# ucsdarclab/diffco

Hardware: AMD Instinct MI355X
Metric: million collision-score+grad evals/sec, 7-DoF FK-kernel, 2k supports (higher is better)
Workload: dtype f32

## Files before the change

diffco_amd/_lib.py:

```python
import ctypes as C
import os

import torch

from ._fkdesc import FkDesc

_HERE = os.path.dirname(os.path.abspath(__file__))
LIB_PATH = os.environ.get("DCX_LIB") or os.path.join(_HERE, "libdcx.so")

_c_fp = C.c_void_p
SYMBOLS = {
    "dcx_version": (C.c_int, []),
    "dcx_last_error": (C.c_char_p, []),
    "dcx_device_count": (C.c_int, []),
    "dcx_debug_set": (C.c_int, [C.c_char_p, C.c_int64]),
    "dcx_debug_clock_probe": (C.c_int, [C.c_int, C.c_void_p, C.c_uint64, C.POINTER(C.c_int32), C.c_void_p]),
    "dcx_model_create": (C.c_int, [C.POINTER(C.c_void_p), C.c_int, C.POINTER(FkDesc), C.c_int, C.POINTER(C.c_float),
                                   _c_fp, _c_fp, C.c_int64, C.c_int32, C.c_int32]),
    "dcx_model_create_ex": (C.c_int, [C.POINTER(C.c_void_p), C.c_int, C.POINTER(FkDesc), C.c_int, C.POINTER(C.c_float),
                                      _c_fp, _c_fp, C.c_int64, C.c_int32, C.c_int32, C.c_int64, C.c_void_p]),
    "dcx_model_update": (C.c_int, [C.c_void_p, _c_fp, _c_fp, C.c_int64, C.c_void_p]),
    "dcx_model_destroy": (None, [C.c_void_p]),
    "dcx_model_info": (C.c_int, [C.c_void_p, C.POINTER(C.c_int64), C.POINTER(C.c_int32), C.POINTER(C.c_int32),
                                 C.POINTER(C.c_int32), C.POINTER(C.c_int32)]),
    "dcx_score": (C.c_int, [C.c_void_p, _c_fp, C.c_int64, _c_fp, C.c_void_p]),
    "dcx_score_grad": (C.c_int, [C.c_void_p, _c_fp, C.c_int64, _c_fp, _c_fp, _c_fp, C.c_void_p]),
    "dcx_score_jac": (C.c_int, [C.c_void_p, _c_fp, C.c_int64, _c_fp, _c_fp, C.c_void_p]),
    "dcx_score_hess": (C.c_int, [C.c_void_p, _c_fp, C.c_int64, _c_fp, _c_fp, _c_fp, C.c_void_p]),
    "dcx_score_hinge_grad": (C.c_int, [C.c_void_p, _c_fp, C.c_int64, C.c_float, C.c_float, _c_fp, _c_fp, C.c_void_p]),
    "dcx_score_hinge_grad_mc": (C.c_int, [C.c_void_p, _c_fp, C.c_int64, C.POINTER(C.c_float), C.c_float, _c_fp, _c_fp, C.c_void_p]),
    "dcx_traj_adam_run_mc": (C.c_int, [C.c_void_p, C.c_void_p, C.c_void_p, C.POINTER(C.c_float), C.c_int32, C.c_int32, C.c_void_p]),
    "dcx_traj_adam_step_mc": (C.c_int, [C.c_int, C.POINTER(FkDesc), C.c_void_p, C.c_void_p, C.POINTER(C.c_float), C.c_int32, C.c_int32,
                                        C.c_void_p]),
    "dcx_traj_adam_step": (C.c_int, [C.c_int, C.POINTER(FkDesc), C.c_void_p, C.c_void_p, C.c_int32, C.c_void_p]),
    "dcx_traj_adam_run": (C.c_int, [C.c_void_p, C.c_void_p, C.c_void_p, C.c_int32, C.c_int32, C.c_void_p]),
    "dcx_escape_work_bytes": (C.c_size_t, [C.c_void_p, C.c_int64]),
    "dcx_escape_adam": (C.c_int, [C.c_void_p, _c_fp, C.c_int64, _c_fp, C.c_void_p, C.c_void_p, C.c_size_t, _c_fp, C.c_void_p,
                                  C.c_void_p]),
    "dcx_train_perceptron": (C.c_int, [C.c_int, C.c_int, C.POINTER(C.c_float), C.c_float, _c_fp, C.c_int64, C.c_int32, _c_fp,
                                       C.c_int32, _c_fp, _c_fp, _c_fp, C.c_int32, _c_fp, C.c_void_p]),
    "dcx_train_perceptron_ex": (C.c_int, [C.c_int, C.c_int, C.POINTER(C.c_float), C.c_float, _c_fp, C.c_int64, C.c_int32, _c_fp,
                                          C.c_int32, _c_fp, _c_fp, _c_fp, C.c_int32, _c_fp, C.c_int32, C.c_void_p]),
    "dcx_fkine": (C.c_int, [C.c_int, C.POINTER(FkDesc), _c_fp, C.c_int64, _c_fp, C.c_void_p]),
    "dcx_fkine_vjp": (C.c_int, [C.c_int, C.POINTER(FkDesc), _c_fp, _c_fp, C.c_int64, _c_fp, C.c_void_p]),
    "dcx_dh_frames": (C.c_int, [C.c_int, _c_fp, C.c_int64, C.c_int32, _c_fp, _c_fp, _c_fp, _c_fp, _c_fp, C.c_void_p]),
    "dcx_dh_frames_vjp": (C.c_int, [C.c_int, _c_fp, C.c_int64, C.c_int32, _c_fp, _c_fp, _c_fp, _c_fp, _c_fp, C.c_void_p]),
    "dcx_euler_frames": (C.c_int, [C.c_int, _c_fp, C.c_int64, _c_fp, C.c_void_p]),
    "dcx_euler_frames_vjp": (C.c_int, [C.c_int, _c_fp, _c_fp, C.c_int64, _c_fp, C.c_void_p]),
    "dcx_kernel_matrix": (C.c_int, [C.c_int, C.c_int, C.POINTER(C.c_float), _c_fp, C.c_int64, _c_fp, C.c_int64,
                                    C.c_int32, _c_fp, C.c_void_p]),
    "dcx_motion_work_bytes": (C.c_size_t, [C.c_void_p, C.c_int64]),
    "dcx_check_motions": (C.c_int, [C.c_void_p, _c_fp, _c_fp, C.c_int64, C.c_void_p, _c_fp, _c_fp, _c_fp, C.c_void_p, C.c_size_t,
                                    C.c_void_p]),
    "dcx_motion_cost_work_bytes": (C.c_size_t, [C.c_void_p, C.c_int64, C.c_int32]),
    "dcx_motion_cost": (C.c_int, [C.c_void_p, _c_fp, _c_fp, C.c_int64, C.c_void_p, _c_fp, C.c_float, _c_fp, _c_fp, _c_fp, _c_fp,
                                  C.c_void_p, C.c_size_t, C.c_void_p]),
    "dcx_solve_work_bytes": (C.c_size_t, [C.c_int64, C.c_int64]),
    "dcx_solve": (C.c_int, [C.c_int, _c_fp, _c_fp, C.c_int64, C.c_int64, _c_fp, C.c_void_p, C.c_size_t, C.c_void_p, C.c_int32,
                            C.c_void_p]),
}



class TrajState(C.Structure):
    _fields_ = [("n_paths", C.c_int32), ("n_waypoints", C.c_int32)] + [
        (n, C.c_void_p) for n in ("path", "adam_m", "adam_v", "limits", "col_score", "col_grad", "stats", "lowest_loss",
                                  "lowest_obj", "lowest_path", "best_valid_obj", "best_valid_path", "done", "steps")]

# ... 67 lines not shown
```

diffco_amd/csrc/dcx_api.hip:

```cpp
#include <algorithm>
#include <atomic>
#include <cmath>
#include <cstdio>
#include <cstdlib>
#include <cstring>
#include <mutex>
#include <new>
#include <string>
#include <vector>

#include "dcx_internal.h"
#include "motion_cost_kernel.h"
#include "motion_kernel.h"
#include "pack_kernels.h"
#include "solve_kernels.h"

using namespace dcx;

struct dcx_model {
    int device = 0;
    dcx_fk_desc fk{};
    FkProg* fk_dev = nullptr;
    DhProg* dh_dev = nullptr;
    DhArgs dh{};
// ... 182 lines not shown
}

int set_device(int device) {
    int n = 0;
    hipError_t e = hipGetDeviceCount(&n);
    if (e != hipSuccess || n == 0) return fail(DCX_ERR_NO_DEVICE, "no HIP device visible (libdcx has no CPU path)");
    if (device < 0 || device >= n) return fail(DCX_ERR_INVALID, "device index out of range");
    DCX_HIP(hipSetDevice(device));
    return DCX_OK;
}

struct FkCacheEntry {
    int device;
    dcx_fk_desc host;
    FkProg* dev;
};
thread_local std::vector<FkCacheEntry> g_fk_cache;

int upload_fk_prog(const dcx_fk_desc& fk, FkProg** out) {
    FkProg prog;
    build_fk_prog(fk, prog);
    FkProg* d = nullptr;
    DCX_HIP(hipMalloc((void**)&d, sizeof(FkProg)));
    hipError_t e = hipMemcpy(d, &prog, sizeof(FkProg), hipMemcpyHostToDevice);
    if (e != hipSuccess) {
        (void)hipFree(d);
        return fail_hip(e, "upload of the FK program");
    }
    *out = d;
    return DCX_OK;
}

int fk_device_copy(int device, const dcx_fk_desc& fk, FkProg** out) {
    for (auto& e : g_fk_cache)
        if (e.device == device && std::memcmp(&e.host, &fk, sizeof(fk)) == 0) {
            *out = e.dev;
            return DCX_OK;
        }
    FkProg* d = nullptr;
    if (int rc = upload_fk_prog(fk, &d)) return rc;
    if (g_fk_cache.size() >= 64) {
        (void)hipFree(g_fk_cache.front().dev);
        g_fk_cache.erase(g_fk_cache.begin());
    }
    g_fk_cache.push_back({device, fk, d});
    *out = d;
    return DCX_OK;
}

struct Knobs {
    std::atomic<int64_t> ys{-1}, nw{-1}, min_rows{-1}, split_finish_kernel{-1}, inlaunch_tiles{-1}, jac_per_class{-1},
        traj_fused{-1}, xf{-1}, jac_one_sweep{-1}, train_grid{-1}, fkk{-1}, jt_waves{-1}, hess_ys{-1}, hess_form{-1},
        traj_ys{-1}, traj_across{-1}, owner_poll{-1}, solve_threads{-1}, qt{-1}, giveup_inject{-1}, skew{-1}, skew8{-1},
        motion_early_exit{-1};
    Knobs() {
        auto rd = [](const char* name, std::atomic<int64_t>& dst, bool flag) {
            if (const char* e = std::getenv(name)) dst = flag ? 1 : std::atoll(e);
        };
        rd("DCX_YS", ys, false);
        rd("DCX_NW", nw, false);
        rd("DCX_MIN_ROWS", min_rows, false);
        rd("DCX_SPLIT_FINISH_KERNEL", split_finish_kernel, true);
        rd("DCX_INLAUNCH_TILES", inlaunch_tiles, false);
        rd("DCX_JAC_PER_CLASS", jac_per_class, true);
        rd("DCX_TRAJ_FUSED", traj_fused, false);
        rd("DCX_XF", xf, false);
        rd("DCX_JAC_ONE_SWEEP", jac_one_sweep, false);
        rd("DCX_TRAIN_GRID", train_grid, false);
        rd("DCX_FKK", fkk, false);
        rd("DCX_JT_WAVES", jt_waves, false);
        rd("DCX_HESS_YS", hess_ys, false);
        rd("DCX_HESS_FORM", hess_form, false);
        rd("DCX_TRAJ_YS", traj_ys, false);
        rd("DCX_TRAJ_ACROSS", traj_across, false);
        rd("DCX_OWNER_POLL", owner_poll, false);
        rd("DCX_SOLVE_THREADS", solve_threads, false);
        rd("DCX_QT", qt, false);
        rd("DCX_SKEW", skew, false);
        rd("DCX_SKEW8", skew8, false);
    }
};
Knobs& knobs() {
    static Knobs k;
    return k;
}

struct Geometry {
    int nw, ys;
    int red_slots;
};
Geometry pick_geometry(const dcx_model* m, int64_t B, int acc_floats, bool allow_split) {
    const int cap = m->max_threads / 64;
    const int64_t tiles = (B + 63) / 64;
    Geometry g;
    g.ys = 1;
    if (allow_split && 2 * tiles <= m->n_cu) {
        const int64_t want = std::min<int64_t>((int64_t)m->n_cu / tiles, m->S_active / 250);
        while (2 * g.ys <= want && g.ys < 32) g.ys *= 2;
        g.nw = std::min(16, cap);
    } else if (allow_split && 3 * tiles <= 2 * (int64_t)m->n_cu && (int64_t)m->S_active * m->Dt >= 18000) {
        g.ys = 3;
        g.nw = std::min(16, cap);
    } else {
        g.nw = std::min((tiles <= 4 * (int64_t)m->n_cu) ? 16 : 8, cap);
    }
    const Knobs& kn = knobs();
    if (const int64_t v = kn.ys; v >= 1 && allow_split) g.ys = (int)std::min<int64_t>(v, 64);
    if (const int64_t v = kn.nw; v >= 1) g.nw = (int)std::min<int64_t>(v, cap);
    int min_rows = 15;
    if (const int64_t v = kn.min_rows; v >= 1) min_rows = (int)v;
    while (g.ys > 1 && m->S_active / (g.ys * g.nw) < min_rows) g.ys /= 2;
    while (g.nw > 1 && m->S_active / (g.ys * g.nw) < min_rows) g.nw /= 2;
    const int d_fk = m->fk.n_points * m->fk.point_dim;
    auto lds_bytes = [&](int nw, int slots) {
        return (size_t)(lds_plan(m->fk.dof, d_fk, m->frame_floats, nw > 1 ? slots : 0, acc_floats, true).total + m->prog_floats) * sizeof(float);
    };
    g.red_slots = g.nw;
    const size_t lds_cap = (g.ys > 1 ? 150 : 64) * 1024;
    if (lds_bytes(g.nw, g.nw) > lds_cap && g.nw >= 8 && lds_bytes(g.nw / 2, g.nw / 2) <= lds_cap && kn.nw < 1) {
        g.nw /= 2;
        g.red_slots = g.nw;
    }
    if (lds_bytes(g.nw, g.nw) > lds_cap) {
        const int wps = sweep_min_waves(m->Dt, m->Cc, m->kf);
        int best_nw = 1, best_waves = 0;
        for (int nw = g.nw; nw >= 1; nw /= 2) {
            const size_t lds = lds_bytes(nw, 1);
            if (lds > 64 * 1024) continue;
            const int by_lds = (int)((160 * 1024) / lds), by_regs = std::max(1, (4 * wps) / nw);
            const int waves = std::min(by_lds, by_regs) * nw;
            if (waves > best_waves) {
                best_waves = waves;
                best_nw = nw;
            }
        }
        g.nw = best_nw;
        g.red_slots = 1;
    }
// ... 92 lines not shown
    }
    m->hess_mom.push_back({st, p, bytes});
    return p;
}

inline int32_t skew_rule(int Cc = 1, bool score_only = false, bool traj = false) {
    const int64_t k = knobs().skew;
    if (k >= 0) return (int32_t)k;
    if (traj && Cc > 1) return 340 | (300 << 10) | (240 << 20);
    if (score_only) return 320 | (300 << 10) | (240 << 20);
    return Cc > 1 ? (420 | (300 << 10) | (200 << 20)) : (480 | (320 << 10) | (150 << 20));
}

inline int32_t skew8_rule(bool score_only = false) {
    const int64_t k = knobs().skew8;
    if (k >= 0) return -(int32_t)k;
    if (score_only) return -540;
    return -600;
}

void set_fk_walk(const dcx_model* m, ScoreArgs& a) {
    a.fk = m->fk_dev;
    a.fk_dwords = m->fk_dwords;
    a.dh = m->dh;
    a.fkk = 0;
    if (m->fk.kind == DCX_FK_DH) {
        const int64_t k = knobs().fkk;
        a.fkk = (k == 0) ? 0 : (k == 1) ? 1 : (m->dh_dev ? 2 : 1);
    }
}

struct Hinge {
    int on = 0;
    float margin = 0.f, weight = 0.f;
    float margin_c[DCX_MAX_C] = {0.f, 0.f, 0.f, 0.f, 0.f, 0.f, 0.f, 0.f};
    int traj_slices = 0;
};

int run_score(const dcx_model* m, const float* q, int64_t B, const float* upstream, float* score, float* grad,
              int mode, int one_hot, int64_t grad_stride, hipStream_t st, Hinge hinge = Hinge(), int nz = 1) {
    if (B == 0) return DCX_OK;
    const int d_fk = m->fk.n_points * m->fk.point_dim;
    const int acc = (mode == MODE_SCORE ? 0 : m->Dt) + m->Cc;
    int64_t nblk = (B + 63) / 64;
    const bool xf_able = knobs().xf != 0 && xf_applies(m->Dt, m->Cc, m->kf) && m->rows_xf_dev != nullptr &&
                         (m->kf != KF_RQ2 || m->xf_rq_ok || knobs().xf >= 2);
    constexpr int QT_SLICES = kQtSlices;
    Geometry g{};
    bool qt = false;
    int qt_per = 0;
    size_t qt_lds = 0;
    const Knobs& kn0 = knobs();
    const bool asked_otherwise = kn0.ys >= 1 || kn0.xf >= 0 || kn0.owner_poll >= 0 || kn0.split_finish_kernel > 0 ||
                                 kn0.inlaunch_tiles >= 0 || kn0.min_rows >= 1;
    if (const int64_t kq = kn0.qt; kq != 0 && (kq > 0 || !asked_otherwise) && qt_applies(m->Dt, m->Cc, m->kf, mode) && nz == 1 &&
                                   m->S_active >= 64 && B <= 16LL * m->n_cu) {
        int nw = std::min(16, m->max_threads / 64);
        if (const int64_t v = knobs().nw; v >= 2) nw = (int)std::min<int64_t>(v, m->max_threads / 64);
        const int nw_rule = nw;
        for (; nw >= 4; nw /= 2) {
            qt_per = (m->S_active + QT_SLICES * nw - 1) / (QT_SLICES * nw);
            const size_t plan = lds_plan(m->fk.dof, d_fk, m->frame_floats, nw, acc, true).total + m->prog_floats;
            qt_lds = sizeof(float) * (((plan + 3) & ~(size_t)3) + (size_t)QT_SLICES * nw * (qt_per * row_stride(m->Dt, m->Cc) + 4) +
                                      (size_t)(12 * m->dh.n_pt + 1) * 64);
            if (qt_lds <= 156 * 1024 && qt_per >= 2) break;
            if (kq < 0) { nw = 0; break; }
        }
        if (nw >= 4 && (kq > 0 || nw == nw_rule)) {
            qt = true;
            g.nw = nw;
            g.ys = 1;
            g.red_slots = nw;
        }
    }
    if (!qt) g = pick_geometry(m, B * nz, acc, true);
    float* part = nullptr;
    uint32_t ptag = 0;
    if (knobs().giveup_inject > 0 && m->giveup_host) {
        knobs().giveup_inject = -1;
        *m->giveup_host = 1;
    }
    if (m->giveup_host && *m->giveup_host)
        return fail(DCX_ERR_HIP, "an earlier split launch of this model gave up waiting for its peer workgroups (owner-polls hand-over: "
                                 "they were never scheduled - the GPU is shared with another process?); its results were NaN. "
                                 "dcx_debug_set(\"owner_poll\", 0) selects the hand-over that never waits");
    if (g.ys > 1) {
        part = split_scratch(m, st, (size_t)nblk * nz * g.ys * acc * 64 * sizeof(float), &ptag);
        if (!part) g = pick_geometry(m, B * nz, acc, false);
    }
    unsigned int* counters = nullptr;
    if (part) {
        const bool second_launch = knobs().split_finish_kernel > 0;
        int64_t inlaunch_max = 256;
        if (const int64_t v = knobs().inlaunch_tiles; v >= 0) inlaunch_max = std::min<int64_t>(v, (int64_t)kTileCounters);
        if (nblk * nz <= inlaunch_max && !second_launch) counters = reinterpret_cast<unsigned int*>(part);
        part = reinterpret_cast<float*>(reinterpret_cast<char*>(part) + kScratchHead);
    }
    if (nblk > 0x7fffffffLL) return fail(DCX_ERR_UNSUPPORTED, "batch too large for one launch");
    ScoreArgs a{};
    a.rows = m->rows_dev;
    set_fk_walk(m, a);
    a.q = q;
    a.upstream = upstream;
    a.score = score;
    a.grad = grad;
    a.B = B;
    a.S = m->S_active;
// ... 11 lines not shown
    a.red_slots = g.red_slots;
    a.dof = m->fk.dof;
    a.d_fk = d_fk;
    a.frame_floats = m->frame_floats;
    a.kind = m->kind;
    a.c_out = m->C;
    a.one_hot = one_hot;
    a.nz = nz;
    a.grad_stride = grad_stride;
    a.kp0 = m->kp0_sweep;
    a.kp1 = m->kp1;
    a.hinge = hinge.on;
    a.hinge_margin = hinge.margin;
    a.hinge_weight = hinge.weight;
    for (int c = 0; c < DCX_MAX_C; ++c) a.hinge_margin_c[c] = hinge.margin_c[c];
    a.xf = xf_able ? 1 : 0;
    if (qt) {
        a.xf = 0;
        a.qt = 1;
        a.qt_per = qt_per;
        for (int gq = 0; gq < 4; ++gq) a.qt_per_g[gq] = qt_per;
        if (g.nw == 16 && skew_rule() > 0) {
            const int32_t sk = skew_rule();
            const int w3[3] = {sk & 1023, (sk >> 10) & 1023, (sk >> 20) & 1023};
            int left = 4 * qt_per;
            for (int gq = 0; gq < 3; ++gq) {
                a.qt_per_g[gq] = std::min(left, (int)((int64_t)4 * qt_per * w3[gq] / 1000));
                left -= a.qt_per_g[gq];
            }
            a.qt_per_g[3] = left;
        }
        a.qt_off = (int32_t)((lds_plan(a.dof, d_fk, m->frame_floats, g.nw, acc, true).total + m->prog_floats + 3) & ~3);
        a.qt_scr = a.qt_off + QT_SLICES * g.nw * (qt_per * row_stride(m->Dt, m->Cc) + 4);
        const int64_t kq = knobs().qt;
        a.qt_front = (int32_t)((int64_t)QT_SLICES * g.nw * qt_per * (kq >= 100 ? std::min<int64_t>(kq - 100, 100) : 45) / 100);
        nblk = (B + 15) / 16;
    }
    if (a.xf) {
        a.rows = m->rows_xf_dev;
        a.centre = m->centre_dev;
    }
    a.jt_rows = (a.fkk == 2 && g.nw >= 2 * m->dh.n_chains && m->dh.n_chains <= 2 && m->dh.end0 <= kDhUnroll &&
                 m->dh.n_steps - m->dh.end0 <= kDhUnroll && knobs().jt_waves != 0) ? 1 : 0;
    a.jt_waves = (a.jt_rows && mode != MODE_SCORE && g.red_slots == g.nw && (g.nw - 1) * acc >= 12 * m->dh.n_pt + 1 &&
                  (g.ys == 1 || counters != nullptr)) ? 1 : 0;
#ifdef DCX_TIMING
    if (!g_ts_dev && hipMalloc((void**)&g_ts_dev, sizeof(unsigned long long) * kTsWords) == hipSuccess)
        (void)hipMemset(g_ts_dev, 0, sizeof(unsigned long long) * kTsWords);
    a.ts = g_ts_dev;
    a.ts_block = std::getenv("DCX_TS_BLOCK") ? (unsigned)std::atoi(std::getenv("DCX_TS_BLOCK")) : 0u;
#endif
    size_t lds = sizeof(float) * (lds_plan(a.dof, d_fk, m->frame_floats, g.nw > 1 ? g.red_slots : 0, acc, true).total + m->prog_floats);
    if (qt) lds = qt_lds;
    if (g.ys == 1) {
        hipError_t e = m->launch(m->kf, m->Cc, mode, g.nw, lds, nblk, a, st);
        if (e != hipSuccess) return fail_hip(e, "score kernel launch");
        return DCX_OK;
    }
    if (nz > 1 && counters == nullptr) return DCX_ERR_UNSUPPORTED;
    a.partial = part;
    a.tile_done = counters;
    if (counters != nullptr && g.red_slots == g.nw && g.nw > 1 && knobs().owner_poll != 0 && (acc <= 2 * g.nw || knobs().owner_poll > 0) &&
        nblk * nz * g.ys <= (int64_t)m->n_cu && 2 * nblk * nz <= (int64_t)m->n_cu && m->giveup_dev != nullptr &&
        (knobs().owner_poll > 0 || opoll_stream_ok(m->device, st))) {
        a.pwords = reinterpret_cast<unsigned long long*>(reinterpret_cast<char*>(part) + (size_t)2 * m->n_cu * (m->Dt + m->Cc) * 64 * sizeof(float));
        a.ptag = ptag;
        a.giveup = m->giveup_dev;
    }
    hipError_t e = m->launch(m->kf, m->Cc, mode, g.nw, lds, nblk, a, st);
    if (e == hipSuccess && counters == nullptr) {
        FinishArgs f{};
        f.partial = part;
        f.fk = m->fk_dev;
        f.q = q;
        f.upstream = (m->C == 1) ? upstream : nullptr;
        f.score = score;
        f.grad = grad;
        f.B = B;
        f.grad_stride = grad_stride;
        f.ys = g.ys;
        f.acc = acc;
        f.C = m->Cc;
        f.c_out = m->C;
        f.Dt = m->Dt;
        f.dof = m->fk.dof;
        f.d_fk = d_fk;
        f.frame_floats = m->frame_floats;
        f.want_grad = (mode != MODE_SCORE);
        f.hinge = hinge.on;
        f.hinge_margin = hinge.margin;
        f.hinge_weight = hinge.weight;
        e = launch_score_finish(f, nblk, sizeof(float) * (lds_plan(a.dof, d_fk, m->frame_floats, 0, 0).total + m->prog_floats), st);
    }
    if (e != hipSuccess) return fail_hip(e, "split score launch");
    return DCX_OK;
}

}

extern "C" {

#ifdef DCX_TIMING
int dcx_debug_ts_words(void) { return (int)kTsWords; }
int dcx_debug_read_ts(unsigned long long* out) {
    if (!g_ts_dev) return 1;
    (void)hipDeviceSynchronize();
    return hipMemcpy(out, g_ts_dev, sizeof(unsigned long long) * kTsWords, hipMemcpyDeviceToHost) == hipSuccess ? 0 : 3;
}
#endif

int dcx_version(void) { return DCX_VERSION; }

int dcx_debug_set(const char* name, int64_t value) {
    if (!name) return fail(DCX_ERR_INVALID, "knob name is NULL");
    Knobs& k = knobs();
    const std::string n(name);
    if (n == "mfma" || n == "xm")
        return value > 0 ? fail(DCX_ERR_UNSUPPORTED, "the matrix-core forms of the sweep were removed (measured slower, profiles/r03_mfma_ab.txt)")
                         : DCX_OK;
    std::atomic<int64_t>* dst = n == "ys" ? &k.ys : n == "nw" ? &k.nw : n == "min_rows" ? &k.min_rows
        : n == "split_finish_kernel" ? &k.split_finish_kernel : n == "inlaunch_tiles" ? &k.inlaunch_tiles
        : n == "jac_per_class" ? &k.jac_per_class : n == "traj_fused" ? &k.traj_fused : n == "xf" ? &k.xf : n == "jac_one_sweep" ? &k.jac_one_sweep : n == "train_grid" ? &k.train_grid : n == "fkk" ? &k.fkk : n == "jt_waves" ? &k.jt_waves : n == "hess_ys" ? &k.hess_ys : n == "hess_form" ? &k.hess_form : n == "traj_ys" ? &k.traj_ys : n == "traj_across" ? &k.traj_across : n == "owner_poll" ? &k.owner_poll : n == "solve_threads" ? &k.solve_threads : n == "qt" ? &k.qt : n == "giveup_inject" ? &k.giveup_inject : n == "skew" ? &k.skew : n == "skew8" ? &k.skew8 : n == "motion_early_exit" ? &k.motion_early_exit : nullptr;
    if (!dst) return fail(DCX_ERR_INVALID, "unknown knob: " + n);
    *dst = value;
    return DCX_OK;
}

const char* dcx_last_error(void) { return g_err.c_str(); }

int dcx_device_count(void) {
    int n = 0;
    if (hipGetDeviceCount(&n) != hipSuccess) return 0;
    return n;
}

static constexpr double kXfRqRule = 32.0;
static size_t rows_tail_floats(const dcx_model* m) { return 8 * (size_t)m->RS + 16; }

static void model_free_rows(dcx_model* m) {
    if (m->rows_dev) (void)hipFree(m->rows_dev);
    if (m->rows_xf_dev) (void)hipFree(m->rows_xf_dev);
    if (m->rows_p2_dev) (void)hipFree(m->rows_p2_dev);
    m->rows_dev = m->rows_xf_dev = m->rows_p2_dev = nullptr;
    m->cap = 0;
}

static int model_alloc_rows(dcx_model* m, int64_t cap) {
    if (cap < 1) cap = 1;
    if (cap <= m->cap && m->rows_dev) return DCX_OK;
    const size_t floats = (size_t)cap * m->RS + rows_tail_floats(m);
    float *rows = nullptr, *rows_xf = nullptr, *rows_p2 = nullptr;
    hipError_t e = hipMalloc((void**)&rows, floats * sizeof(float));
    if (e == hipSuccess) e = hipMalloc((void**)&rows_xf, floats * sizeof(float));
    if (e == hipSuccess && p2_applies(m->Dt, m->Cc, m->kf)) e = hipMalloc((void**)&rows_p2, (floats + m->RS) * sizeof(float));
    if (e == hipSuccess && !m->centre_dev) e = hipMalloc((void**)&m->centre_dev, (size_t)m->Dt * sizeof(float));
    if (e == hipSuccess && !m->info_dev) e = hipMalloc((void**)&m->info_dev, 16);
    if (e == hipSuccess && !m->info_host) e = hipHostMalloc((void**)&m->info_host, 16, hipHostMallocDefault);
    if (e == hipSuccess && !m->giveup_host) {
        e = hipHostMalloc((void**)&m->giveup_host, sizeof(int32_t), hipHostMallocMapped);
        if (e == hipSuccess) {
            *m->giveup_host = 0;
            e = hipHostGetDevicePointer((void**)&m->giveup_dev, m->giveup_host, 0);
        }
    }
    if (e != hipSuccess) {
        if (rows) (void)hipFree(rows);
        if (rows_xf) (void)hipFree(rows_xf);
        if (rows_p2) (void)hipFree(rows_p2);
        return fail_hip(e, "device allocation of the model");
    }
    model_free_rows(m);
    m->rows_dev = rows;
    m->rows_xf_dev = rows_xf;
    m->rows_p2_dev = rows_p2;
    m->cap = cap;
    return DCX_OK;
}
// ... 1155 lines not shown
```

diffco_amd/csrc/score_inst.hip:

```cpp
#include "dcx_internal.h"
#include "traj_fused.h"
#include "jac_kernel.h"

#ifndef DCX_INST_D
#error "compile with -DDCX_INST_D=<feature width>"
#endif

#if (defined(DCX_STUB) && DCX_INST_PART != 0) || (DCX_INST_PART == 2 && DCX_INST_D > 24)
#elif defined(DCX_STUB)
namespace dcx {
#define DCX_CAT_(a, b) a##b
#define DCX_CAT(a, b) DCX_CAT_(a, b)
hipError_t DCX_CAT(launch_score_D, DCX_INST_D)(int, int, int, int, size_t, int64_t, const ScoreArgs&, hipStream_t) { return hipErrorNotSupported; }
hipError_t DCX_CAT(launch_jac_D, DCX_INST_D)(int, int, int, size_t, int64_t, const ScoreArgs&, hipStream_t) { return hipErrorNotSupported; }
hipError_t DCX_CAT(launch_traj_fused_D, DCX_INST_D)(int, int, int, size_t, int, const TrajFusedArgs&, hipStream_t) { return hipErrorNotSupported; }
}
#else
namespace dcx {
namespace {

constexpr int kD = DCX_INST_D;
constexpr int kMaxT = kD <= 16 ? 1024 : (kD <= 48 ? 512 : 256);


template <int KF, int CC, int MODE>
hipError_t go(int nw, size_t lds, int64_t nblk, const ScoreArgs& a, hipStream_t st) {
    const dim3 grid((unsigned)nblk, (unsigned)(a.ys > 1 ? a.ys : 1), (unsigned)(a.nz > 1 ? a.nz : 1));
    auto launch = [&](auto kern) {
        if (lds > 64 * 1024) {
            hipError_t e = hipFuncSetAttribute((const void*)kern, hipFuncAttributeMaxDynamicSharedMemorySize, (int)lds);
            if (e != hipSuccess) return e;
        }
        kern<<<grid, dim3(64 * nw), lds, st>>>(a);
        return hipGetLastError();
    };
    if constexpr (qt_applies(kD, CC, KF, MODE)) {
        if (a.qt) return launch(score_kernel<kD, KF, CC, MODE, kMaxT, false, true>);
    }
    if constexpr (xf_applies(kD, CC, KF)) {
        if (a.xf) return launch(score_kernel<kD, KF, CC, MODE, kMaxT, true>);
    }
    return launch(score_kernel<kD, KF, CC, MODE, kMaxT>);
}

template <int KF, int CC>
hipError_t by_mode(int mode, int nw, size_t lds, int64_t nblk, const ScoreArgs& a, hipStream_t st) {
    switch (mode) {
    case MODE_SCORE: return go<KF, CC, MODE_SCORE>(nw, lds, nblk, a, st);
    case MODE_GRAD_ROW: return go<KF, CC, MODE_GRAD_ROW>(nw, lds, nblk, a, st);
    case MODE_GRAD_UP:
        if constexpr (CC > 1) return go<KF, CC, MODE_GRAD_UP>(nw, lds, nblk, a, st);
    default: return hipErrorInvalidValue;
    }
}

template <int KF>
hipError_t by_cc(int cc, int mode, int nw, size_t lds, int64_t nblk, const ScoreArgs& a, hipStream_t st) {
    switch (cc) {
    case 1: return by_mode<KF, 1>(mode, nw, lds, nblk, a, st);
    case 5: return by_mode<KF, 5>(mode, nw, lds, nblk, a, st);
#ifndef DCX_DEV_FAST
    case 4: return by_mode<KF, 4>(mode, nw, lds, nblk, a, st);
    case 8: return by_mode<KF, 8>(mode, nw, lds, nblk, a, st);
#endif
    default: return hipErrorInvalidValue;
    }
}

}

#define DCX_CAT_(a, b) a##b
#define DCX_CAT(a, b) DCX_CAT_(a, b)
#ifndef DCX_INST_PART
#error "compile with -DDCX_INST_PART=0, 1 and (D <= 24) 2"
#endif
hipError_t DCX_CAT(launch_score_gen_D, DCX_INST_D)(int cc, int mode, int nw, size_t lds, int64_t nblk, const ScoreArgs& a, hipStream_t st);
namespace {
template <class K>
hipError_t traj_go(K kern, int nw, size_t lds, int n_paths, const TrajFusedArgs& a, hipStream_t st) {
    if (lds > 64 * 1024) {
        hipError_t e = hipFuncSetAttribute((const void*)kern, hipFuncAttributeMaxDynamicSharedMemorySize, (int)lds);
        if (e != hipSuccess) return e;
    }
    if (a.ys > 1) {
        TrajFusedArgs copy = a;
        void* params[] = {&copy};
        const dim3 grid = a.cl_across ? dim3((unsigned)a.ys, (unsigned)n_paths) : dim3((unsigned)n_paths, (unsigned)a.ys);
        return hipLaunchCooperativeKernel((const void*)kern, grid, dim3(64 * nw), params, (unsigned int)lds, st);
// ... 135 lines not shown
```

diffco_amd/csrc/score_kernel.h:

```cpp
#pragma once
#include <hip/hip_runtime.h>
#include <type_traits>
#include <stdint.h>
#include "fk_device.h"

namespace dcx {

enum { KF_RQ2 = 0,
       KF_POLY1 = 1,
       KF_GEN = 2 };

enum { MODE_SCORE = 0,
       MODE_GRAD_ROW = 1,
       MODE_GRAD_UP = 2 };

struct ScoreArgs {
    const float* rows;
    const float* centre;
    const FkProg* fk;
    const float* q;
    const float* upstream;
    float* score;
    float* grad;
    int64_t B;
    int32_t S;
    int32_t s_chunk;
    int32_t dof;
    int32_t d_fk;
    int32_t frame_floats;
    int32_t kind;
    int32_t c_out;
    int32_t one_hot;
    int32_t nz;
    int64_t grad_stride;
    float* partial;
    unsigned int* tile_done;
    unsigned long long* pwords;
    uint32_t ptag;
    int32_t* giveup;
    int32_t ys;
    int32_t s_super;
    int32_t red_slots;
#ifdef DCX_TIMING
    unsigned long long* ts;
    unsigned int ts_block;
#endif
    float kp0, kp1;
    int32_t xf;
    int32_t fkk;
    int32_t fk_dwords;
    DhArgs dh;
    int32_t jt_rows;
    int32_t jt_waves;
    int32_t hinge;
    float hinge_margin, hinge_weight;
    float hinge_margin_c[8];
    int32_t s_skew;
    int32_t qt;
    int32_t qt_off;
    int32_t qt_per;
    int32_t qt_per_g[4];
    int32_t qt_scr;
    int32_t qt_front;
};

#ifndef DCX_ROW_ALIGN_MULTI
#define DCX_ROW_ALIGN_MULTI 4
#endif
template <int D, int CC>
struct RowLayout {
    static constexpr int W_OFF = D;
    static constexpr int WSUM_OFF = D + CC;
    static constexpr int SS_OFF = D + CC + (CC > 1 ? 1 : 0);
    static constexpr int AL = CC > 1 ? DCX_ROW_ALIGN_MULTI : 4;
    static constexpr int RS = (SS_OFF + 1 + AL - 1) / AL * AL;
};

__device__ __forceinline__ void wave_slice(int wave, int nw, int s_chunk, int skew, int ybase, int yend, int& j0, int& j1) {
    int start = wave * s_chunk, len = s_chunk;
    if (skew > 0 && nw == 16) {
        const int w0 = skew & 1023, w1 = (skew >> 10) & 1023, w2 = (skew >> 20) & 1023;
        const int l0 = (s_chunk * w0 / 250) & ~1, l1 = (s_chunk * w1 / 250) & ~1, l2 = (s_chunk * w2 / 250) & ~1;
        int l3 = 4 * s_chunk - l0 - l1 - l2;
        l3 = l3 > 0 ? l3 : 0;
        const int g = wave >> 2, q = wave & 3;
        len = (g == 0) ? l0 : (g == 1) ? l1 : (g == 2) ? l2 : l3;
        start = 4 * ((g > 0 ? l0 : 0) + (g > 1 ? l1 : 0) + (g > 2 ? l2 : 0)) + q * len;
    } else if (skew < 0 && nw == 8) {
        int l0 = (s_chunk * (-skew) / 500) & ~1;
        l0 = l0 < 2 * s_chunk ? l0 : 2 * s_chunk;
        const int g = wave >> 2, q = wave & 3;
        len = g ? 2 * s_chunk - l0 : l0;
        start = (g ? 4 * l0 : 0) + q * len;
    }
    j0 = (ybase + start < yend) ? ybase + start : yend;
    j1 = (j0 + len < yend) ? j0 + len : yend;
}

constexpr int kCounterStride = 32;

typedef const __attribute__((address_space(4))) float* cfloat_ptr;
typedef float v2f __attribute__((ext_vector_type(2)));

#ifdef DCX_TIMING
#define DCX_TS(slot)                                                                              \
    do {                                                                                          \
        if (a.ts && blockIdx.x == a.ts_block && blockIdx.y == 0 && (threadIdx.x & 63) == 0 && (threadIdx.x >> 6) < 16) \
            a.ts[(slot) * 16 + (threadIdx.x >> 6)] = __builtin_readcyclecounter();               \
    } while (0)
#define DCX_TSB(k)                                                                                 \
    do {                                                                                           \
        const unsigned bl__ = blockIdx.x + gridDim.x * blockIdx.y;                                \
        if (a.ts && bl__ < 4096 && threadIdx.x == 0) {                                             \
            unsigned long long t__ = __builtin_readcyclecounter();                                 \
            if ((k) == 0) {                                                                        \
                unsigned hw__, xcc__;                                                              \
// ... 1249 lines not shown
                }
            }
#pragma unroll
            for (int u = 0; u < 4; ++u)
                if (e0 + u < ACC) sRed[(e0 + u) * 64 + lane] = tot[u];
        }
#pragma unroll
        for (int c = 0; c < CC; ++c) sc[c] = sRed[c * 64 + lane];
        if constexpr (GRAD) {
#pragma unroll
            for (int k = 0; k < D; ++k) gx[k] = sRed[(CC + k) * 64 + lane];
        }
    }

    if (b.score != nullptr && lane < nb && blockIdx.z == 0) {
#pragma unroll
        for (int c = 0; c < CC; ++c)
            if (c < b.c_out) b.score[(b0 + lane) * b.c_out + c] = sc[c];
    }
    }

    if constexpr (GRAD) {
        float scale = 1.0f;
        if constexpr (CC == 1 && MODE == MODE_GRAD_ROW) {
            if (b.upstream != nullptr) scale = b.upstream[b0 + (lane < nb ? lane : nb - 1)];
            if (b.hinge) scale = (sc[0] - b.hinge_margin > 0.0f) ? b.hinge_weight : 0.0f;
        }
        if (b.d_fk == D) {
#pragma unroll
            for (int k = 0; k < D; ++k) sG[k * 64 + lane] = gx[k] * scale;
        } else {
#pragma unroll
            for (int k = 0; k < D; ++k)
                if (k < b.d_fk) sG[k * 64 + lane] = gx[k] * scale;
        }
        DCX_FK_TS(12, 2);
        float* gq = smem + lp.q;
        fk_vjp_sel(fw, dhb, sQ + lane * dof, sF + lane, sG + lane, gq + lane * dof, dof);
        DCX_TS(5);
        __builtin_amdgcn_fence(__ATOMIC_ACQ_REL, "workgroup");
        __builtin_amdgcn_wave_barrier();
        float* gdst = b.grad + b0 * b.grad_stride + (b.nz > 1 ? (size_t)blockIdx.z * dof : 0);
        const int n = nb * dof;
        if (b.grad_stride == dof) {
            for (int i = lane; i < n; i += 64) gdst[i] = gq[i];
        } else {
            for (int i = lane; i < n; i += 64) gdst[(int64_t)(i / dof) * b.grad_stride + (i % dof)] = gq[i];
        }
        DCX_TSB(3);
    }
    }
}

struct FinishArgs {
    const float* partial;
    const FkProg* fk;
    const float* q;
    const float* upstream;
    float* score;
    float* grad;
    int64_t B;
    int64_t grad_stride;
    int32_t ys, acc, C, Dt, dof, d_fk, frame_floats, want_grad;
    int32_t c_out;
    int32_t hinge;
    float hinge_margin, hinge_weight;
};

}
```

include/dcx.h:

```cpp
#ifndef DCX_H
#define DCX_H

#include <stddef.h>
#include <stdint.h>

#ifdef __cplusplus
extern "C" {
#endif

#define DCX_VERSION 109

#define DCX_OK 0
#define DCX_ERR_INVALID 1
#define DCX_ERR_UNSUPPORTED 2
#define DCX_ERR_HIP 3
#define DCX_ERR_NO_DEVICE 4

#define DCX_K_RQ 0
#define DCX_K_POLY 1
#define DCX_K_MQ 2

#define DCX_FK_NONE 0
#define DCX_FK_PLANAR 1
#define DCX_FK_DH 2
// ... 9 lines not shown

#define DCX_MAX_JOINTS 16
#define DCX_MAX_CHAINS 2
#define DCX_MAX_POINTS 32
#define DCX_MAX_DOF 32
#define DCX_MAX_D 96
#define DCX_MAX_C 8
#define DCX_MAX_TREE_CHAINS 16
#define DCX_MAX_TREE_BASES 4
#define DCX_MAX_TREE_JOINTS 64

typedef struct dcx_fk_desc {
    int32_t kind;
    int32_t dof;
    int32_t n_points;
    int32_t point_dim;

    float link_length[DCX_MAX_DOF];

    int32_t n_chains;
    int32_t chain_len[DCX_MAX_CHAINS];
    int32_t joint_q[DCX_MAX_CHAINS][DCX_MAX_JOINTS];
    float a[DCX_MAX_CHAINS][DCX_MAX_JOINTS];
    float d[DCX_MAX_CHAINS][DCX_MAX_JOINTS];
    float sin_alpha[DCX_MAX_CHAINS][DCX_MAX_JOINTS];
    float cos_alpha[DCX_MAX_CHAINS][DCX_MAX_JOINTS];
    float theta0[DCX_MAX_CHAINS][DCX_MAX_JOINTS];
    float base[DCX_MAX_CHAINS][12];
    int32_t pt_chain[DCX_MAX_POINTS];
    int32_t pt_frame[DCX_MAX_POINTS];
    float pt_off[DCX_MAX_POINTS][3];

    float keypoints[DCX_MAX_POINTS][3];

    int32_t t_n_chains;
    int32_t t_coord_major;
    int32_t t_chain_len[DCX_MAX_TREE_CHAINS];
    float t_base[DCX_MAX_TREE_CHAINS][12];
    int32_t t_type[DCX_MAX_TREE_JOINTS];
    int32_t t_q[DCX_MAX_TREE_JOINTS];
    float t_scale[DCX_MAX_TREE_JOINTS];
    float t_offset[DCX_MAX_TREE_JOINTS];
    float t_fixed[DCX_MAX_TREE_JOINTS][12];
    float t_axis[DCX_MAX_TREE_JOINTS][3];
} dcx_fk_desc;

typedef struct dcx_model dcx_model;

int dcx_version(void);
const char* dcx_last_error(void);
int dcx_device_count(void);

int dcx_debug_set(const char* name, int64_t value);
int dcx_debug_clock_probe(int device, uint64_t* out4, uint64_t wall_ticks, int32_t* wall_clock_khz, void* stream);

int dcx_model_create(dcx_model** out, int device, const dcx_fk_desc* fk, int kernel_kind,
                     const float* kparams, const float* support_feat, const float* weights,
                     int64_t S, int32_t D, int32_t C);
int dcx_model_create_ex(dcx_model** out, int device, const dcx_fk_desc* fk, int kernel_kind,
                        const float* kparams, const float* support_feat, const float* weights,
                        int64_t S, int32_t D, int32_t C, int64_t capacity, void* stream);
int dcx_model_update(dcx_model* m, const float* support_feat, const float* weights, int64_t S, void* stream);
void dcx_model_destroy(dcx_model* m);
int dcx_model_info(const dcx_model* m, int64_t* S_active, int32_t* D, int32_t* C, int32_t* dof,
                   int32_t* device);

int dcx_score(const dcx_model* m, const float* q, int64_t B, float* score, void* stream);

int dcx_score_grad(const dcx_model* m, const float* q, int64_t B, const float* upstream,
                   float* score, float* grad, void* stream);

int dcx_score_jac(const dcx_model* m, const float* q, int64_t B, float* score, float* jac,
                  void* stream);

int dcx_score_hess(const dcx_model* m, const float* q, int64_t B, const float* upstream, float* grad, float* hess,
                   void* stream);

int dcx_score_hinge_grad(const dcx_model* m, const float* q, int64_t B, float margin, float weight,
                         float* score, float* grad, void* stream);
int dcx_score_hinge_grad_mc(const dcx_model* m, const float* q, int64_t B, const float* margin, float weight,
                            float* score, float* grad, void* stream);

typedef struct dcx_traj_state {
    int32_t n_paths, n_waypoints;
    float* path;
    float* adam_m;
    float* adam_v;
    const float* limits;
    const float* col_score;
    const float* col_grad;
    float* stats;
    float* lowest_loss;
    float* lowest_obj;
    float* lowest_path;
    float* best_valid_obj;
    float* best_valid_path;
    int32_t* done;
    int32_t* steps;
} dcx_traj_state;

typedef struct dcx_traj_opts {
    float lr, beta1, beta2, eps;
    float w_diff, w_collision, w_max_move, w_joint_limit;
    float safety_margin, max_speed;
    float valid_tol, grad_tol;
} dcx_traj_opts;
// ... 75 lines not shown
```

Baseline: 763.8.

## Add two-tile score kernel processing 128 configs per block

```diff
diff --git a/diffco_amd/_lib.py b/diffco_amd/_lib.py
--- a/diffco_amd/_lib.py
+++ b/diffco_amd/_lib.py
@@ -14,6 +14,7 @@
     "dcx_last_error": (C.c_char_p, []),
     "dcx_device_count": (C.c_int, []),
     "dcx_debug_set": (C.c_int, [C.c_char_p, C.c_int64]),
+    "dcx_debug_get": (C.c_int, [C.c_char_p, C.POINTER(C.c_int64)]),
     "dcx_debug_clock_probe": (C.c_int, [C.c_int, C.c_void_p, C.c_uint64, C.POINTER(C.c_int32), C.c_void_p]),
     "dcx_model_create": (C.c_int, [C.POINTER(C.c_void_p), C.c_int, C.POINTER(FkDesc), C.c_int, C.POINTER(C.c_float),
                                    _c_fp, _c_fp, C.c_int64, C.c_int32, C.c_int32]),
diff --git a/diffco_amd/csrc/dcx_api.hip b/diffco_amd/csrc/dcx_api.hip
--- a/diffco_amd/csrc/dcx_api.hip
+++ b/diffco_amd/csrc/dcx_api.hip
@@ -258,7 +258,7 @@
     std::atomic<int64_t> ys{-1}, nw{-1}, min_rows{-1}, split_finish_kernel{-1}, inlaunch_tiles{-1}, jac_per_class{-1},
         traj_fused{-1}, xf{-1}, jac_one_sweep{-1}, train_grid{-1}, fkk{-1}, jt_waves{-1}, hess_ys{-1}, hess_form{-1},
         traj_ys{-1}, traj_across{-1}, owner_poll{-1}, solve_threads{-1}, qt{-1}, giveup_inject{-1}, skew{-1}, skew8{-1},
-        motion_early_exit{-1};
+        motion_early_exit{-1}, tile2{-1};
     Knobs() {
         auto rd = [](const char* name, std::atomic<int64_t>& dst, bool flag) {
             if (const char* e = std::getenv(name)) dst = flag ? 1 : std::atoll(e);
@@ -284,12 +284,14 @@
         rd("DCX_QT", qt, false);
         rd("DCX_SKEW", skew, false);
         rd("DCX_SKEW8", skew8, false);
+        rd("DCX_TILE2", tile2, false);
     }
 };
 Knobs& knobs() {
     static Knobs k;
     return k;
 }
+std::atomic<int64_t> g_last_tile2{0};
 
 struct Geometry {
     int nw, ys;
@@ -488,7 +490,7 @@
     size_t qt_lds = 0;
     const Knobs& kn0 = knobs();
     const bool asked_otherwise = kn0.ys >= 1 || kn0.xf >= 0 || kn0.owner_poll >= 0 || kn0.split_finish_kernel > 0 ||
-                                 kn0.inlaunch_tiles >= 0 || kn0.min_rows >= 1;
+                                 kn0.inlaunch_tiles >= 0 || kn0.min_rows >= 1 || kn0.tile2 >= 0;
     if (const int64_t kq = kn0.qt; kq != 0 && (kq > 0 || !asked_otherwise) && qt_applies(m->Dt, m->Cc, m->kf, mode) && nz == 1 &&
                                    m->S_active >= 64 && B <= 16LL * m->n_cu) {
         int nw = std::min(16, m->max_threads / 64);
@@ -606,6 +608,26 @@
 #endif
     size_t lds = sizeof(float) * (lds_plan(a.dof, d_fk, m->frame_floats, g.nw > 1 ? g.red_slots : 0, acc, true).total + m->prog_floats);
     if (qt) lds = qt_lds;
+    g_last_tile2 = 0;
+    if (const int64_t kt = kn0.tile2; kt != 0 && !qt && g.ys == 1 && nz == 1 && g.nw == 16 && g.red_slots == 16 && a.fkk == 2 &&
+                                      a.jt_rows && 4 * m->dh.n_chains <= 16 && (mode == MODE_SCORE || a.jt_waves)) {
+        constexpr int64_t kT2MaxRounds = 2;
+        const int64_t resident = 2 * (int64_t)m->n_cu;
+        const bool others = kn0.ys >= 1 || kn0.xf >= 0 || kn0.owner_poll >= 0 || kn0.split_finish_kernel > 0 || kn0.inlaunch_tiles >= 0 ||
+                            kn0.min_rows >= 1 || kn0.nw >= 1 || kn0.qt >= 0;
+        const int off = (int)((lds / sizeof(float) + 63) & ~(size_t)63);
+        const T2Lds tp = t2_lds(off, a.dof, d_fk, m->frame_floats, m->dh.n_pt, mode != MODE_SCORE);
+        const int jb_last = m->dh.n_chains > 1 ? m->dh.end0 : 0;
+        const int over = std::max(0, 2 * (jb_last + kDhUnroll) - m->frame_floats) * 64;
+        const size_t lds2 = sizeof(float) * (size_t)(off + std::max(tp.total, tp.j - off + over));
+        if ((kt > 0 || (!others && nblk >= 2 * resident && nblk <= kT2MaxRounds * resident)) && 2 * lds2 <= 160 * 1024) {
+            a.tile2 = 1;
+            a.t2_off = off;
+            lds = lds2;
+            nblk = (nblk + 1) / 2;
+            g_last_tile2 = 1;
+        }
+    }
     if (g.ys == 1) {
         hipError_t e = m->launch(m->kf, m->Cc, mode, g.nw, lds, nblk, a, st);
         if (e != hipSuccess) return fail_hip(e, "score kernel launch");
@@ -674,9 +696,18 @@
                          : DCX_OK;
     std::atomic<int64_t>* dst = n == "ys" ? &k.ys : n == "nw" ? &k.nw : n == "min_rows" ? &k.min_rows
         : n == "split_finish_kernel" ? &k.split_finish_kernel : n == "inlaunch_tiles" ? &k.inlaunch_tiles
-        : n == "jac_per_class" ? &k.jac_per_class : n == "traj_fused" ? &k.traj_fused : n == "xf" ? &k.xf : n == "jac_one_sweep" ? &k.jac_one_sweep : n == "train_grid" ? &k.train_grid : n == "fkk" ? &k.fkk : n == "jt_waves" ? &k.jt_waves : n == "hess_ys" ? &k.hess_ys : n == "hess_form" ? &k.hess_form : n == "traj_ys" ? &k.traj_ys : n == "traj_across" ? &k.traj_across : n == "owner_poll" ? &k.owner_poll : n == "solve_threads" ? &k.solve_threads : n == "qt" ? &k.qt : n == "giveup_inject" ? &k.giveup_inject : n == "skew" ? &k.skew : n == "skew8" ? &k.skew8 : n == "motion_early_exit" ? &k.motion_early_exit : nullptr;
+        : n == "jac_per_class" ? &k.jac_per_class : n == "traj_fused" ? &k.traj_fused : n == "xf" ? &k.xf : n == "jac_one_sweep" ? &k.jac_one_sweep : n == "train_grid" ? &k.train_grid : n == "fkk" ? &k.fkk : n == "jt_waves" ? &k.jt_waves : n == "hess_ys" ? &k.hess_ys : n == "hess_form" ? &k.hess_form : n == "traj_ys" ? &k.traj_ys : n == "traj_across" ? &k.traj_across : n == "owner_poll" ? &k.owner_poll : n == "solve_threads" ? &k.solve_threads : n == "qt" ? &k.qt : n == "giveup_inject" ? &k.giveup_inject : n == "skew" ? &k.skew : n == "skew8" ? &k.skew8 : n == "motion_early_exit" ? &k.motion_early_exit : n == "tile2" ? &k.tile2 : nullptr;
     if (!dst) return fail(DCX_ERR_INVALID, "unknown knob: " + n);
     *dst = value;
+    return DCX_OK;
+}
+
+int dcx_debug_get(const char* name, int64_t* value) {
+    if (!name || !value) return fail(DCX_ERR_INVALID, "dcx_debug_get: NULL argument");
+    const std::string n(name);
+    if (n == "last_tile2") *value = g_last_tile2;
+    else if (n == "tile2") *value = knobs().tile2;
+    else return fail(DCX_ERR_INVALID, "unknown readable: " + n);
     return DCX_OK;
 }
 
diff --git a/diffco_amd/csrc/score_inst.hip b/diffco_amd/csrc/score_inst.hip
--- a/diffco_amd/csrc/score_inst.hip
+++ b/diffco_amd/csrc/score_inst.hip
@@ -34,6 +34,16 @@
         kern<<<grid, dim3(64 * nw), lds, st>>>(a);
         return hipGetLastError();
     };
+    if constexpr (kMaxT == 1024) {
+        if (a.tile2) {
+            if constexpr (xf_applies(kD, CC, KF)) {
+                if (a.xf) return launch(score_kernel_t2<kD, KF, CC, MODE, kMaxT, true>);
+            }
+            return launch(score_kernel_t2<kD, KF, CC, MODE, kMaxT>);
+        }
+    } else if (a.tile2) {
+        return hipErrorNotSupported;
+    }
     if constexpr (qt_applies(kD, CC, KF, MODE)) {
         if (a.qt) return launch(score_kernel<kD, KF, CC, MODE, kMaxT, false, true>);
     }
diff --git a/diffco_amd/csrc/score_kernel.h b/diffco_amd/csrc/score_kernel.h
--- a/diffco_amd/csrc/score_kernel.h
+++ b/diffco_amd/csrc/score_kernel.h
@@ -62,6 +62,8 @@
     int32_t qt_per_g[4];
     int32_t qt_scr;
     int32_t qt_front;
+    int32_t tile2;
+    int32_t t2_off;
 };
 
 #ifndef DCX_ROW_ALIGN_MULTI
@@ -1417,6 +1419,178 @@
     }
 }
 
+struct T2Lds {
+    int x, f, j, total;
+};
+__host__ __device__ inline T2Lds t2_lds(int off, int dof, int d_fk, int frame_floats, int n_pt, bool grad) {
+    T2Lds p;
+    p.x = off;
+    p.f = p.x + 64 * d_fk;
+    p.j = p.f + 64 * frame_floats;
+    const int r1 = grad ? 64 * 9 * n_pt : 0, qf = (64 * dof + 3) & ~3;
+    p.total = p.j + (r1 > qf ? r1 : qf) - off;
+    return p;
+}
+
+template <int D, int KF, int CC, int MODE, int MAXT, bool XF = false>
+__global__ __launch_bounds__(MAXT, sweep_min_waves(D, CC, KF)) void score_kernel_t2(const ScoreArgs a) {
+    extern __shared__ __attribute__((aligned(16))) float smem[];
+    constexpr bool GRAD = (MODE != MODE_SCORE);
+    constexpr int ACC = (GRAD ? D : 0) + CC;
+    constexpr int NW = 16;
+    {
+        const int lane = threadIdx.x & 63;
+        const int wave = __builtin_amdgcn_readfirstlane(threadIdx.x >> 6);
+        const int64_t b0 = (int64_t)blockIdx.x * 128;
+        const int64_t left = a.B - b0;
+        const int nb0 = left < 64 ? (int)left : 64;
+        const int nb1 = left > 64 ? (left < 128 ? (int)(left - 64) : 64) : 0;
+        const int dof = a.dof;
+        const LdsPlan lp = lds_plan(dof, a.d_fk, a.frame_floats, NW, ACC, true);
+        const T2Lds tp = t2_lds(a.t2_off, dof, a.d_fk, a.frame_floats, a.dh.n_pt, GRAD);
+        float* sQ0 = smem + lp.q;
+        float* sQ1 = smem + tp.j;
+        const FkWalk fw = fk_stage_sel(a.fkk, a.fk, a.fk_dwords, a.dh, smem + lp.fk, threadIdx.x, blockDim.x);
+        {
+            const float* qsrc = a.q + b0 * dof;
+            const int n0 = nb0 * dof, n1 = nb1 * dof;
+            for (int i = threadIdx.x; i < 64 * dof; i += blockDim.x) sQ0[i] = qsrc[i < n0 ? i : (i % dof) + (nb0 - 1) * dof];
+            if (nb1 > 0)
+                for (int i = threadIdx.x; i < 64 * dof; i += blockDim.x) sQ1[i] = qsrc[64 * dof + (i < n1 ? i : (i % dof) + (nb1 - 1) * dof)];
+        }
+        __syncthreads();
+        fk_trig_sel(fw, a.dh, sQ0 + lane * dof, smem + lp.f + lane, wave, NW);
+        if (nb1 > 0) fk_trig_sel(fw, a.dh, sQ1 + lane * dof, smem + tp.f + lane, (wave + NW / 2) & (NW - 1), NW);
+        __syncthreads();
+        const int cw = 2 * a.dh.n_chains;
+        if (wave < cw) dh2_chain_rows_sel(fw.dh, a.dh, smem + lp.x + lane, smem + lp.f + lane, wave);
+        else if (nb1 > 0 && wave < 2 * cw) dh2_chain_rows_sel(fw.dh, a.dh, smem + tp.x + lane, smem + tp.f + lane, wave - cw);
+        __syncthreads();
+        if constexpr (GRAD) {
+            if (nb1 > 0 && wave >= NW - cw) dh2_vjp_r1_sel(fw.dh, a.dh, smem + tp.f + lane, smem + tp.j + lane, wave - (NW - cw), 9);
+        }
+    }
+    auto run_tile = [&](auto tc) __attribute__((always_inline)) {
+        constexpr int tt = decltype(tc)::value;
+        float x[D];
+        float up[CC];
+        float sc[CC];
+        float gx[D];
+        int j0, j1;
+        {
+            const auto& p = reload_args();
+            const int lane = fresh_lane();
+            const int wave = __builtin_amdgcn_readfirstlane(threadIdx.x >> 6);
+            const int64_t b0 = (int64_t)blockIdx.x * 128 + 64 * tt;
+            if (tt > 0 && b0 >= p.B) return;
+            const int nb = (int)((p.B - b0) < 64 ? (p.B - b0) : 64);
+            const float* sX = smem + (tt ? p.t2_off : 0);
+            if (p.d_fk == D) {
+#pragma unroll
+                for (int k = 0; k < D; ++k) x[k] = sX[k * 64 + lane];
+            } else {
+#pragma unroll
+                for (int k = 0; k < D; ++k) x[k] = (k < p.d_fk) ? sX[k * 64 + lane] : 0.0f;
+            }
+            if constexpr (XF) {
+                cfloat_ptr cen = (cfloat_ptr)(uintptr_t)p.centre;
+#pragma unroll
+                for (int k = 0; k < D; ++k) x[k] -= cen[k];
+            }
+            __syncthreads();
+            if constexpr (MODE == MODE_GRAD_UP) {
+                const int64_t bl = b0 + (lane < nb ? lane : nb - 1);
+                const int hot = p.one_hot;
+#pragma unroll
+                for (int c = 0; c < CC; ++c) up[c] = (hot >= 0) ? (c == hot ? 1.0f : 0.0f) : (c < p.c_out ? p.upstream[bl * p.c_out + c] : 0.0f);
+                if (p.hinge == 2) {
+#pragma unroll
+                    for (int c = 0; c < CC; ++c) up[c] = (c < p.c_out && up[c] - p.hinge_margin_c[c < 8 ? c : 7] > 0.0f) ? p.hinge_weight : 0.0f;
+                }
+            }
+#pragma unroll
+            for (int c = 0; c < CC; ++c) sc[c] = 0.0f;
+#pragma unroll
+            for (int k = 0; k < D; ++k) gx[k] = 0.0f;
+            wave_slice(wave, NW, p.s_chunk, p.s_skew, 0, p.S, j0, j1);
+        }
+        sweep_rows<D, KF, CC, MODE, XF>(a, x, up, j0, j1, sc, gx);
+        {
+            const auto& b = reload_args();
+            const int lane = fresh_lane();
+            const int wave = __builtin_amdgcn_readfirstlane(threadIdx.x >> 6);
+            const int64_t b0 = (int64_t)blockIdx.x * 128 + 64 * tt;
+            const int nb = (int)((b.B - b0) < 64 ? (b.B - b0) : 64);
+            const int dof = b.dof;
+            const LdsPlan lp = lds_plan(dof, b.d_fk, b.frame_floats, NW, ACC, true);
+            float* sRed = smem + lp.red;
+            float* mine = sRed + (size_t)wave * ACC * 64 + lane;
+#pragma unroll
+            for (int c = 0; c < CC; ++c) mine[c * 64] = sc[c];
+            if constexpr (GRAD) {
+#pragma unroll
+                for (int k = 0; k < D; ++k) mine[(CC + k) * 64] = gx[k];
+            }
+            __syncthreads();
+            for (int e = wave; e < ACC; e += NW) {
+                float r[NW];
+#pragma unroll
+                for (int w = 0; w < NW; ++w) r[w] = sRed[((size_t)w * ACC + e) * 64 + lane];
+                float v = r[0];
+#pragma unroll
+                for (int w = 1; w < NW; ++w) v += r[w];
+                sRed[e * 64 + lane] = v;
+            }
+            __syncthreads();
+            if (wave == 0 && b.score != nullptr && lane < nb) {
+#pragma unroll
+                for (int c = 0; c < CC; ++c)
+                    if (c < b.c_out) b.score[(b0 + lane) * b.c_out + c] = sRed[c * 64 + lane];
+            }
+            if constexpr (GRAD) {
+                DhArgs dhb;
+                DCX_COPY_DH(dhb, b.dh);
+                const dh_cptr dhp = (dh_cptr)(uintptr_t)(uint32_t)(uintptr_t)(smem + lp.fk);
+                float scale = 1.0f;
+                if constexpr (CC == 1 && MODE == MODE_GRAD_ROW) {
+                    if (b.upstream != nullptr) scale = b.upstream[b0 + (lane < nb ? lane : nb - 1)];
+                    if (b.hinge) scale = (sRed[lane] - b.hinge_margin > 0.0f) ? b.hinge_weight : 0.0f;
+                }
+                float* gq = smem + lp.q;
+                if constexpr (tt == 0) {
+                    float* scr = sRed + (size_t)ACC * 64 + lane;
+                    dh2_vjp_r1_sel(dhp, dhb, smem + lp.f + lane, scr, wave);
+                    __syncthreads();
+                    dh2_vjp_r1b(dhp, dhb, sRed + CC * 64 + lane, scale, scr, gq + lane * dof, dof, wave, NW);
+                    __syncthreads();
+                    dh2_vjp_r2_sel(dhp, dhb, smem + lp.f + lane, scr, gq + lane * dof, wave);
+                } else {
+                    const T2Lds tp = t2_lds(b.t2_off, dof, b.d_fk, b.frame_floats, dhb.n_pt, true);
+                    float* scr = smem + tp.j + lane;
+                    const int loff = (lp.red - tp.j) / 64 + ACC;
+                    dh2_vjp_r1b(dhp, dhb, sRed + CC * 64 + lane, scale, scr, gq + lane * dof, dof, wave, NW, 9, loff);
+                    __syncthreads();
+                    dh2_vjp_r2_sel(dhp, dhb, smem + tp.f + lane, scr, gq + lane * dof, wave, 9, loff);
+                }
+                if (dhb.n_chains > 1 && !dhb.shared_q) __syncthreads();
+                if (wave == 0) {
+                    __builtin_amdgcn_fence(__ATOMIC_ACQ_REL, "workgroup");
+                    __builtin_amdgcn_wave_barrier();
+                    float* gdst = b.grad + b0 * b.grad_stride;
+                    const int n = nb * dof;
+                    if (b.grad_stride == dof) {
+                        for (int i = lane; i < n; i += 64) gdst[i] = gq[i];
+                    } else {
+                        for (int i = lane; i < n; i += 64) gdst[(int64_t)(i / dof) * b.grad_stride + (i % dof)] = gq[i];
+                    }
+                }
+            }
+        }
+    };
+    run_tile(std::integral_constant<int, 0>{});
+    run_tile(std::integral_constant<int, 1>{});
+}
+
 struct FinishArgs {
     const float* partial;
     const FkProg* fk;
diff --git a/include/dcx.h b/include/dcx.h
--- a/include/dcx.h
+++ b/include/dcx.h
@@ -85,6 +85,7 @@
 int dcx_device_count(void);
 
 int dcx_debug_set(const char* name, int64_t value);
+int dcx_debug_get(const char* name, int64_t* value);
 int dcx_debug_clock_probe(int device, uint64_t* out4, uint64_t wall_ticks, int32_t* wall_clock_khz, void* stream);
 
 int dcx_model_create(dcx_model** out, int device, const dcx_fk_desc* fk, int kernel_kind,
```

After: 747.8. -2.1%, worse.
